# lightkurve/lightkurve

Hardware: NVIDIA H100
Metric: lombscargle_freqbins_x_cadences_per_s (higher is better)
Workload: dtype f32 spreading + FFT, f64 phase (nufft)

## Files before the change

lightkurve_b200/csrc/ls_nufft.cu:

```cuda
#include <algorithm>

#include "common.cuh"
#include "ls_common.cuh"
#include "nufft_core.h"
#include "nufft_v2.cuh"

namespace lkb {

using nufft::Cad;

namespace {

constexpr int GL_NQ = 48;
struct GlNodes {
  double x[GL_NQ], w[GL_NQ];
};

__global__ void nufft_cad_kernel(const double* __restrict__ t, int64_t N, double df, int64_t M, int w,
                                 Cad* __restrict__ cad, int* __restrict__ unsorted) {
  const int64_t n = (int64_t)blockIdx.x * blockDim.x + threadIdx.x;
  if (n >= N) return;
  cad[n] = nufft::cad_entry(t[n], df, M, w);
  if (n > 0 && t[n] < t[n - 1]) *unsorted = 1;
  if (t[n] < 0.0) *unsorted = 1;
// ... 307 lines not shown
    for (int64_t s0 = n_lo; s0 < n_hi; s0 += 256) {
      float v0[8], v1[8];
#pragma unroll
      for (int q = 0; q < 8; ++q) {
        const int64_t n = s0 + lane + 32 * q;
        v0[q] = (n < n_hi) ? y0[n] : 0.0f;
        v1[q] = (n < n_hi) ? y1[n] : 0.0f;
      }
      __syncthreads();
      {
        const int64_t n = s0 + threadIdx.x;
#pragma unroll
        for (int r = 0; r < LOWR; ++r)
          sD[r][threadIdx.x] = (r < nr && n < n_hi) ? D[(int64_t)(r0 + r) * Npad + n] : make_float2(0.f, 0.f);
      }
      __syncthreads();
#pragma unroll
      for (int q = 0; q < 8; ++q) {
#pragma unroll
        for (int r = 0; r < LOWR; ++r) {
          const float2 d = sD[r][lane + 32 * q];
          ac0[r] = fmaf(v0[q], d.x, ac0[r]); as0[r] = fmaf(v0[q], d.y, as0[r]);
          ac1[r] = fmaf(v1[q], d.x, ac1[r]); as1[r] = fmaf(v1[q], d.y, as1[r]);
        }
      }
    }
#pragma unroll
    for (int r = 0; r < LOWR; ++r) {
      if (r < nr) {
        const double c0v = warp_sum((double)ac0[r]), s0v = warp_sum((double)as0[r]);
        const double c1v = warp_sum((double)ac1[r]), s1v = warp_sum((double)as1[r]);
        if (lane == 0) {
          if (b0 < B) { atomicAdd(acc + ((int64_t)b0 * F_low + r0 + r) * 2, c0v); atomicAdd(acc + ((int64_t)b0 * F_low + r0 + r) * 2 + 1, s0v); }
          if (b1 < B) { atomicAdd(acc + ((int64_t)b1 * F_low + r0 + r) * 2, c1v); atomicAdd(acc + ((int64_t)b1 * F_low + r0 + r) * 2 + 1, s1v); }
        }
      }
    }
  }
}
__global__ void nufft2_lowfinish_kernel(const double* __restrict__ acc, int B, int F_low, int64_t F, int64_t N,
                                        const float4* __restrict__ rot, const float2* __restrict__ rot2,
                                        const float* __restrict__ ysum, int normalization, float scale,
                                        float* __restrict__ power, unsigned* __restrict__ peak) {
  const int e = (int)(blockIdx.x * blockDim.x + threadIdx.x);
  if (e >= B * F_low) return;
  const int b = e / F_low, k = e - b * F_low;
  const float pw = ls_epilogue_shared((float)acc[2 * (int64_t)e], (float)acc[2 * (int64_t)e + 1], rot[k], rot2[k], ysum[b],
                                      (float)N, LKB_LS_NORM_PSD_RAW, 1.0f, true);
  power[(int64_t)b * F + k] = v2_normalise(pw, (float)N, normalization, scale);
  if (peak && pw > 0.0f) atomicMax(peak + b, __float_as_uint(pw));
}

constexpr int LOWX_PER = 8;
__global__ void __launch_bounds__(256)
nufft2_lowacc_kernel(const int* __restrict__ list, V2Count nc, const double* __restrict__ t, int64_t N,
                     const float* __restrict__ yc, int64_t ystride, const double* __restrict__ freq, int F_low,
                     double* __restrict__ accW, double* __restrict__ accY, double* __restrict__ accS) {
  const int ntr = v2_count(nc, 0);
  if (ntr <= 0) return;
  const int k = (int)blockIdx.x, lane = threadIdx.x & 31;
  const int64_t n0 = (int64_t)blockIdx.y * (256 * LOWX_PER) + threadIdx.x;
  const double fr = freq[k];
  double sn[LOWX_PER], cs[LOWX_PER];
  double ws = 0.0, wc = 0.0, wcc = 0.0, wsc = 0.0;
#pragma unroll
  for (int q = 0; q < LOWX_PER; ++q) {
    const int64_t n = n0 + (int64_t)q * 256;
    sn[q] = 0.0; cs[q] = 0.0;
    if (n < N) {
      ls_sincos_cycles_f64(fr * t[n], sn[q], cs[q]);
      ws += sn[q]; wc += cs[q]; wcc += cs[q] * cs[q]; wsc += sn[q] * cs[q];
    }
  }
  ws = warp_sum(ws); wc = warp_sum(wc); wcc = warp_sum(wcc); wsc = warp_sum(wsc);
  if (lane == 0) {
    atomicAdd(accW + 4 * k + 0, ws); atomicAdd(accW + 4 * k + 1, wc);
    atomicAdd(accW + 4 * k + 2, wcc); atomicAdd(accW + 4 * k + 3, wsc);
  }
  for (int i = 0; i < ntr; ++i) {
    const float* y = yc + (int64_t)list[nc.base + i] * ystride;
    double sh = 0.0, ch = 0.0, sy = 0.0;
#pragma unroll
    for (int q = 0; q < LOWX_PER; ++q) {
      const int64_t n = n0 + (int64_t)q * 256;
      const double v = (n < N) ? (double)y[n] : 0.0;
      sh = fma(v, sn[q], sh);
      ch = fma(v, cs[q], ch);
      sy += v;
    }
    sh = warp_sum(sh); ch = warp_sum(ch);
    if (k == 0) sy = warp_sum(sy);
    if (lane == 0) {
      atomicAdd(accY + ((int64_t)i * F_low + k) * 2 + 0, sh);
      atomicAdd(accY + ((int64_t)i * F_low + k) * 2 + 1, ch);
      if (k == 0) atomicAdd(accS + i, sy);
    }
  }
}
__global__ void nufft2_lowexact_finish_kernel(const int* __restrict__ list, V2Count nc, const double* __restrict__ accW,
                                              const double* __restrict__ accY, const double* __restrict__ accS,
                                              int F_low, int64_t F, int64_t N, int normalization, float scale,
                                              float* __restrict__ power) {
  const int ntr = v2_count(nc, 0);
  const int e = (int)(blockIdx.x * blockDim.x + threadIdx.x);
  if (e >= ntr * F_low) return;
  const int i = e / F_low, k = e - i * F_low;
  LsSums<double> d;
  d.sh = accY[2 * (int64_t)e]; d.ch = accY[2 * (int64_t)e + 1];
  d.s = accW[4 * k]; d.c = accW[4 * k + 1]; d.cc = accW[4 * k + 2]; d.sc = accW[4 * k + 3];
  power[(int64_t)list[nc.base + i] * F + k] =
      ls_normalize(ls_power_from_sums(d, (double)N, accS[i]), (double)N, normalization, (double)scale);
}

__global__ void __launch_bounds__(128)
nufft2_verify_kernel(const float2* __restrict__ Zn, int p, const float2* __restrict__ dec, int64_t k0, int64_t F,
                     int64_t k_lo, const double* __restrict__ t, int64_t N, const float* __restrict__ yc, int64_t ystride,
                     const double* __restrict__ freq, int nv, float fault, unsigned* __restrict__ worst) {
  const int warp = threadIdx.x >> 5, lane = threadIdx.x & 31;
  const unsigned job = blockIdx.x * (blockDim.x >> 5) + warp;
  unsigned h = job * 2654435761u + 12345u;
  h ^= h >> 15; h *= 2246822519u; h ^= h >> 13;
  const int64_t b = h % (unsigned)nv;
  const int64_t k = k_lo + (int64_t)((h >> 8) % (unsigned)(F - k_lo));
  const float* y = yc + b * ystride;
  const double fr = freq[k];
  double c = 0.0, s = 0.0, l1 = 0.0;
  for (int64_t i = lane; i < N; i += 32) {
    double sn, cs;
    ls_sincos_cycles_f64(fr * t[i], sn, cs);
    const double v = (double)y[i];
    c += v * cs;
    s += v * sn;
    l1 += fabs(v);
  }
  c = warp_sum(c);
  s = warp_sum(s);
  l1 = warp_sum(l1);
  if (lane == 0) {
    const int64_t M = (int64_t)1 << p, Mh = M >> 1, kk = k0 + k;
    const float2 g1 = Zn[b * Mh + kk], g2 = Zn[b * Mh + ((Mh - kk) & (Mh - 1))];
    const float2 E = make_float2(0.5f * (g1.x + g2.x), 0.5f * (g1.y - g2.y));
    const float2 O = make_float2(0.5f * (g1.y + g2.y), 0.5f * (g2.x - g1.x));
    double wsn, wcs;
    sincospi(2.0 * (double)kk / (double)M, &wsn, &wcs);
    const float2 G = make_float2(E.x + (float)wcs * O.x - (float)wsn * O.y, E.y + (float)wcs * O.y + (float)wsn * O.x);
    const float2 got = nufft::cmul(G, dec[k]);
    const double dev = fmax(fabs((double)got.x * (double)fault - c), fabs((double)got.y * (double)fault - s));
    const double units = dev / (1e-7 * fmax(l1, 1e-300));
// ... 273 lines not shown
    LKB_TRY(ws_get_t<float2>(ws_alt ? WS_OUT5 : WS_I, std::max((size_t)B * cells, verify ? (size_t)4 * Mh : (size_t)0), &G));
    unsigned* d_worst = nullptr;
    if (verify) LKB_TRY(ws_get_t<unsigned>(ws_alt ? WS_OUT7 : WS_OUT6, 1, &d_worst));
    const int ptc = V2_LOG_TILE - (p - 1 - V2_PB);
    if (prof) prof_begin(st);
    constexpr int LCS = 8;
    LKB_LAUNCH(dim3(blocks_for((int64_t)cells, 256), (unsigned)((B + LCS - 1) / LCS)), 256, st, nufft2_spread_kernel<LCS>)(
        pl.fge, pl.cad, pl.Wt, d_yc, ystride, B, w, p, ptc, pl.n1max, G);
    LKB_LAUNCH_CHECK();
    LKB_TRY(v2_cols(G, T, p, pl.n1max, B, pl.tb, st));
    const float esc_ratio = escalate_ratio();
    unsigned* d_peak = nullptr;
    int* d_list = nullptr;
    if (esc_ratio > 0.0f && F_low < F) {
      LKB_TRY(ws_get_t<unsigned>(ws_alt ? WS_Y3 : WS_Y2, (size_t)2 * B + 1, &d_peak));
      d_list = reinterpret_cast<int*>(d_peak + B);
      LKB_CUDA_CHECK(cudaMemsetAsync(d_peak, 0, sizeof(unsigned) * ((size_t)B + 1), st));
    }
    V2Finish fa;
    fa.ftab = pl.ftab; fa.k0 = k0; fa.F = F; fa.k_lo = F_low; fa.ysum = d_ysumf; fa.Nf = (float)N;
    fa.normalization = normalization; fa.scale = (float)norm_scale; fa.power = d_pow;
    fa.peak = d_peak; fa.lcmap = nullptr; fa.log2M = p;
    if (F_low < F) LKB_TRY(v2_rows(T, p, B, pl.tb, &fa, (float2*)nullptr, 0, st));
    if (F_low > 0) {
      double* acc = nullptr;
      LKB_TRY(ws_get_t<double>(ws_alt ? WS_X4 : WS_X3, (size_t)B * F_low * 2, &acc));
      LKB_CUDA_CHECK(cudaMemsetAsync(acc, 0, sizeof(double) * (size_t)B * F_low * 2, st));
      const int groups = (B + 15) / 16;
      const int64_t slice = 2048;
      LKB_LAUNCH(dim3((unsigned)groups, (unsigned)((N + slice - 1) / slice)), 256, st, nufft2_lowrows_kernel)(
          pl.lowD, N, pl.Npad, d_yc, ystride, B, (int)F_low, slice, acc);
      LKB_LAUNCH_CHECK();
      LKB_LAUNCH(blocks_for((int64_t)B * F_low, 256), 256, st, nufft2_lowfinish_kernel)(
          acc, B, (int)F_low, F, N, d_rot, d_rot2, d_ysumf, normalization, (float)norm_scale, d_pow, d_peak);
      LKB_LAUNCH_CHECK();
    }
    if (d_peak) {
      LKB_LAUNCH(blocks_for(B, 256), 256, st, nufft2_flag_kernel)(d_peak, d_absmax, B, (float)N, esc_ratio, d_list, d_list + 1,
                                                                pl.esc_total);
      LKB_LAUNCH_CHECK();
      int cap_max = 1024;
      if (const char* e = getenv("LKB_NUFFT_ESCALATE_CAP")) cap_max = std::max(1, atoi(e));
      const int cap = std::min(B, cap_max), gy = std::min(cap, 32);
      const size_t lowlen = F_low > 0 ? (size_t)F_low * 4 + (size_t)cap * F_low * 2 + cap : 0;
      double *Gbuf = nullptr;
      double2* Td = nullptr;
      LKB_TRY(ws_get_t<double>(ws_alt ? WS_Y6 : WS_Y4, 2 * (size_t)cap * cells + lowlen, &Gbuf));
      LKB_TRY(ws_get_t<double2>(ws_alt ? WS_Y7 : WS_Y5, (size_t)cap * Mh, &Td));
      double2* Gd = reinterpret_cast<double2*>(Gbuf);
      double* accW = Gbuf + 2 * (size_t)cap * cells;
      double* accY = accW + (size_t)F_low * 4;
      double* accS = accY + (size_t)cap * F_low * 2;
      const int* lst = d_list + 1;
      for (int base = 0; base < B; base += cap) {
        const V2Count nc = {d_list, base, cap};
        LKB_LAUNCH(dim3(blocks_for((int64_t)cells, 256), (unsigned)gy), 256, st, nufft2_spread_list_kernel)(
            pl.fge, pl.cad, pl.Wtd, d_yc, ystride, lst, w, p, ptc, pl.n1max, Gd, nc);
        LKB_LAUNCH_CHECK();
        LKB_TRY(v2_cols(Gd, Td, p, pl.n1max, gy, pl.tbd, st, nc));
        V2Finish fd = fa;
        fd.peak = nullptr;
        fd.lcmap = lst;
        LKB_TRY(v2_rows(Td, p, gy, pl.tbd, &fd, (double2*)nullptr, 0, st, nc));
        if (F_low > 0) {
          LKB_CUDA_CHECK(cudaMemsetAsync(accW, 0, sizeof(double) * lowlen, st));
          LKB_LAUNCH(dim3((unsigned)F_low, blocks_for(N, 256 * LOWX_PER)), 256, st, nufft2_lowacc_kernel)(
              lst, nc, d_t, N, d_yc, ystride, d_freq, (int)F_low, accW, accY, accS);
          LKB_LAUNCH_CHECK();
          LKB_LAUNCH(blocks_for((int64_t)cap * F_low, 256), 256, st, nufft2_lowexact_finish_kernel)(
              lst, nc, accW, accY, accS, (int)F_low, F, N, normalization, (float)norm_scale, d_pow);
          LKB_LAUNCH_CHECK();
        }
      }
    }
    if (prof) prof_end(st);
    if (verify) {
      const int nv = std::min(B, 4);
      const int nk2 = (int)((k0 + F) >> (p - 1 - V2_PB)) + 1;
      LKB_TRY(v2_rows(T, p, nv, pl.tb, (const V2Finish*)nullptr, G, nk2, st));
      const char* fe = getenv("LKB_NUFFT_INJECT_FAULT");
      LKB_CUDA_CHECK(cudaMemsetAsync(d_worst, 0, sizeof(unsigned), st));
      LKB_LAUNCH(16, 128, st, nufft2_verify_kernel)(G, p, pl.dec, k0, F, F_low, d_t, N, d_yc, ystride, d_freq, nv,
                                                  fe ? (float)atof(fe) : 1.0f, d_worst);
      LKB_LAUNCH_CHECK();
      unsigned h_worst = 0;
      LKB_CUDA_CHECK(cudaMemcpyAsync(&h_worst, d_worst, sizeof(unsigned), cudaMemcpyDeviceToHost, st));
      LKB_CUDA_CHECK(cudaStreamSynchronize(st));
      if (h_worst > 100u) {
        set_error("NUFFT self-check failed: transform deviates from the direct sums by %u x 1e-7 sum|y|", h_worst);
        return LKB_E_VERIFY;
      }
    }
    return LKB_OK;
  }
  float2 *Za = nullptr, *Zb = nullptr;
  LKB_TRY(ws_get_t<float2>(ws_alt ? WS_OUT4 : WS_H, (size_t)npairs * M, &Za));
  LKB_TRY(ws_get_t<float2>(ws_alt ? WS_OUT5 : WS_I, (size_t)npairs * M, &Zb));
  unsigned* d_worst = nullptr;
  if (verify) LKB_TRY(ws_get_t<unsigned>(ws_alt ? WS_OUT7 : WS_OUT6, 1, &d_worst));

  int group = npairs;
  if (const char* e = getenv("LKB_NUFFT_GROUP_MB")) {
    const double mb = atof(e);
    if (mb > 0.0) {
      const double per_pair = 2.0 * (double)M * sizeof(float2) / 1048576.0;
      group = (int)fmax(1.0, floor(mb / per_pair));
      if (group > npairs) group = npairs;
    }
  }
  if (prof) prof_begin(st);
// ... 614 lines not shown
```

lightkurve_b200/csrc/nufft_v2.cuh:

```cuda
#pragma once
#include "nufft_core.h"

namespace lkb {
namespace {

using nufft::V2_PB;
using nufft::V2_THREADS;
using nufft::V2_TILE;
constexpr int V2_LOG_TILE = 13;
static_assert((1 << V2_LOG_TILE) == V2_TILE, "tile size");
constexpr int V2_BC = 1 << V2_PB;
constexpr int V2_R = V2_TILE / (2 * V2_BC);
constexpr int V2_LSB = V2_BC + V2_BC / 16 + 1;
constexpr int V2R_P_MIN = V2_PB + 4 + 1, V2R_P_MAX = V2_PB + 13 + 1;

__host__ __device__ constexpr int v2_radix(int plog, int idx) {
  return (idx < plog / 4) ? 16 : ((idx == plog / 4 && (plog % 4)) ? (1 << (plog % 4)) : 0);
}
__host__ __device__ constexpr int v2_log2i(int r) { return r == 16 ? 4 : r == 8 ? 3 : r == 4 ? 2 : r == 2 ? 1 : 0; }
__device__ __forceinline__ int v2_skew(int a) { return a + (a >> 4); }
template <int nb>
__host__ __device__ constexpr int v2_in_off(int r) {
  return (nb % 16 == 0) ? r * (nb + nb / 16) : r * nb + ((r * nb) >> 4);
}

template <class CT>
__global__ void nufft2_tables_kernel(int pa, int pb, int ph, CT* __restrict__ tw_a, CT* __restrict__ tw_b,
                                     CT* __restrict__ t_hi, CT* __restrict__ t_lo) {
  const int la = nufft::v2_pass_table_len(pa), lb = nufft::v2_pass_table_len(pb), pl = nufft::v2_log2_lo(ph);
  const int nlo = 1 << pl, nhi = 1 << (ph - pl);
  int e = (int)(blockIdx.x * blockDim.x + threadIdx.x);
  int64_t num = 0, den = 1;
  CT* dst = nullptr;
  if (e < la) { nufft::v2_pass_table_entry(pa, e, &num, &den); dst = tw_a + e; }
  else if ((e -= la) < lb) { nufft::v2_pass_table_entry(pb, e, &num, &den); dst = tw_b + e; }
  else if ((e -= lb) < nhi) { num = e; den = nhi; dst = t_hi + e; }
  else if ((e -= nhi) < nlo) { num = e; den = (int64_t)1 << ph; dst = t_lo + e; }
  else return;
  double sn, cs;
  sincospi(2.0 * (double)num / (double)den, &sn, &cs);
  typedef typename nufft::CplxOf<CT>::real RT;
  *dst = nufft::CplxOf<CT>::mk((RT)cs, (RT)sn);
}

template <class RT>
__global__ void nufft2_weights_kernel(const double* __restrict__ t, int64_t N, double df, int64_t M, int w, double beta,
                                      RT* __restrict__ Wt) {
  const int64_t e = (int64_t)blockIdx.x * blockDim.x + threadIdx.x;
  if (e >= N * w) return;
  const int64_t n = e / w;
  const int q = (int)(e - n * w);
  const double x = df * t[n] * (double)M + (double)nufft::grid_shift(w);
  const double i0 = ceil(x - 0.5 * (double)w);
  const double z = (i0 + (double)q - x) * (2.0 / (double)w);
  const double s2 = 1.0 - z * z;
  Wt[e] = (s2 > 0.0) ? (RT)exp(beta * (sqrt(s2) - 1.0)) : (RT)0.0;
}

__device__ __forceinline__ int64_t v2_zcell_of(int64_t e, int ptc, int n1max) {
  const int64_t j = e & (((int64_t)1 << ptc) - 1), rest = e >> ptc;
  const int64_t n1 = rest % n1max, c = rest / n1max;
  return (n1 << V2_PB) + (c << ptc) + j;
}

template <int LCS>
__global__ void __launch_bounds__(256)
nufft2_spread_kernel(const int32_t* __restrict__ first_ge, const nufft::Cad* __restrict__ cad,
                     const float* __restrict__ Wt, const float* __restrict__ y, int64_t ystride, int B, int w, int p,
                     int ptc, int n1max, float2* __restrict__ G) {
  const int64_t cells = (int64_t)n1max << V2_PB;
  const int64_t e = (int64_t)blockIdx.x * blockDim.x + threadIdx.x;
  if (e >= cells) return;
  const int64_t M = (int64_t)1 << p, m = 2 * v2_zcell_of(e, ptc, n1max);
  const int lc0 = (int)blockIdx.y * LCS;
  const float* yr[LCS];
#pragma unroll
  for (int q = 0; q < LCS; ++q) {
    int b = lc0 + q;
    if (b > B - 1) b = B - 1;
    yr[q] = y + (int64_t)b * ystride;
  }
  float a0[LCS], a1[LCS];
#pragma unroll
  for (int q = 0; q < LCS; ++q) { a0[q] = 0.0f; a1[q] = 0.0f; }
  const int64_t L = nufft::table_len(M, w);
  for (int wrap = 0; wrap < 2; ++wrap) {
    const int64_t mm = m + (int64_t)wrap * M;
    if (mm + 1 >= L) break;
    int64_t lo_c = mm - w + 1, hi_c = mm + 2;
    if (lo_c < 0) lo_c = 0;
    if (hi_c > L - 1) hi_c = L - 1;
    const int32_t na = first_ge[lo_c], nb = first_ge[hi_c];
    for (int32_t n = na; n < nb; ++n) {
      const int tap = (int)(mm - (int64_t)cad[n].i0);
      const float* wr = Wt + (int64_t)n * w;
      const float w0 = (tap >= 0) ? wr[tap] : 0.0f;
      const float w1 = (tap + 1 < w) ? wr[tap + 1] : 0.0f;
#pragma unroll
      for (int q = 0; q < LCS; ++q) {
        const float v = yr[q][n];
        a0[q] = fmaf(w0, v, a0[q]);
        a1[q] = fmaf(w1, v, a1[q]);
      }
    }
  }
#pragma unroll
  for (int q = 0; q < LCS; ++q)
    if (lc0 + q < B) G[(int64_t)(lc0 + q) * cells + e] = make_float2(a0[q], a1[q]);
}

template <int PLOG, int LS, int IDX, int NS, class CT = float2>
__device__ __forceinline__ void v2_pass_t(CT* buf, const CT* __restrict__ tw, int nz = 1 << 30) {
  constexpr int R = v2_radix(PLOG, IDX);
  if constexpr (R != 0) {
    constexpr int LR = v2_log2i(R), NB = 16 / R, PNB = PLOG - LR, nb = 1 << PNB;
    constexpr bool WIDE = nb > V2_THREADS;
    static_assert(WIDE || (V2_THREADS % nb) == 0, "geometry");
    const int t = (int)threadIdx.x;
    CT u[NB][R];
    int base_in[NB];
#pragma unroll
    for (int q = 0; q < NB; ++q) {
      int line, i;
      if constexpr (WIDE) { line = 0; i = t + V2_THREADS * q; }
      else { line = (t >> PNB) + ((V2_THREADS * q) >> PNB); i = t & (nb - 1); }
      base_in[q] = line * LS + ((nb % 16 == 0) ? v2_skew(i) : i);
#pragma unroll
      for (int r = 0; r < R; ++r)
        u[q][r] = (IDX > 0 || r * nb < nz) ? buf[base_in[q] + v2_in_off<nb>(r)] : nufft::CplxOf<CT>::mk(0, 0);
    }
    __syncthreads();
#pragma unroll
    for (int q = 0; q < NB; ++q) {
      int line, i;
      if constexpr (WIDE) { line = 0; i = t + V2_THREADS * q; }
      else { line = (t >> PNB) + ((V2_THREADS * q) >> PNB); i = t & (nb - 1); }
      const int k = i & (NS - 1);
      if constexpr (NS > 1) {
#pragma unroll
        for (int r = 1; r < R; ++r) u[q][r] = nufft::cmul(u[q][r], tw[r * NS + k]);
      }
      nufft::SmallDft<R, CT>::run(u[q]);
      const int j = ((i - k) << LR) + k;
      const int base_out = line * LS + ((NS == 1) ? (j + i) : v2_skew(j));
#pragma unroll
      for (int r = 0; r < R; ++r) buf[base_out + ((NS == 1) ? r : r * (NS + NS / 16))] = u[q][r];
    }
    __syncthreads();
    v2_pass_t<PLOG, LS, IDX + 1, NS * R, CT>(buf, tw + ((IDX > 0) ? R * NS : 0));
  }
}

struct V2Count {
  const int* count;
  int base, cap;
};
__device__ __forceinline__ int v2_count(const V2Count nc, int grid_y) {
  if (!nc.count) return grid_y;
  const int n = *nc.count - nc.base;
  return n < 0 ? 0 : (n > nc.cap ? nc.cap : n);
}

template <int PA, class CT>
__device__ __forceinline__ void v2_cols_one(CT* buf, const CT* __restrict__ G, CT* __restrict__ T, int n1max,
                                            const CT* __restrict__ tw_a, const CT* __restrict__ t_hi,
                                            const CT* __restrict__ t_lo, const int64_t lc) {
  constexpr int A = 1 << PA, PTC = V2_LOG_TILE - PA, TC = 1 << PTC, LS = A + A / 16 + 1, C = V2_BC / TC;
  constexpr int JW = TC < 32 ? TC : 32, RW = V2_THREADS / JW, CG = TC / JW;
  constexpr int LJW = JW == 32 ? 5 : JW == 16 ? 4 : JW == 8 ? 3 : JW == 4 ? 2 : JW == 2 ? 1 : 0;
  static_assert((1 << LJW) == JW && RW % 16 == 0, "geometry");
  const int t = (int)threadIdx.x, c = (int)blockIdx.x;
  const int jl = t & (JW - 1), nl = t >> LJW;
  const int nvalid = n1max << PTC;
  const CT* Gp = G + (lc * C + c) * (int64_t)nvalid;
  const int s_base = jl * LS + v2_skew(nl), g_base = nl * TC + jl;
  constexpr int NB1 = A / v2_radix(PA, 0);
  const int nz = ((n1max + NB1 - 1) / NB1) * NB1;
#pragma unroll
  for (int u = 0; u < 16; ++u) {
    const int cg = u % CG, nbk = u / CG;
    if (nbk * RW < nz) {
      const int idx = g_base + nbk * RW * TC + cg * JW;
      buf[s_base + cg * JW * LS + nbk * (RW + RW / 16)] = (idx < nvalid) ? Gp[idx] : nufft::CplxOf<CT>::mk(0, 0);
    }
  }
  __syncthreads();
  v2_pass_t<PA, LS, 0, 1, CT>(buf, tw_a, nz);
  CT* Tp = T + (lc * C + c) * (int64_t)V2_TILE;
  const int ph = PA + V2_PB, pl = nufft::v2_log2_lo(ph);
  const unsigned Mmask = (1u << ph) - 1u, lmask = (1u << pl) - 1u;
#pragma unroll
  for (int u = 0; u < 16; ++u) {
    const int cg = u % CG, nbk = u / CG;
    const int k1 = nl + nbk * RW, n2 = c * TC + jl + cg * JW;
    const unsigned q = ((unsigned)n2 * (unsigned)k1) & Mmask;
    const CT wq = nufft::cmul(t_hi[q >> pl], t_lo[q & lmask]);
    Tp[g_base + nbk * RW * TC + cg * JW] = nufft::cmul(buf[s_base + cg * JW * LS + nbk * (RW + RW / 16)], wq);
  }
}
template <int PA, class CT = float2>
__global__ void __launch_bounds__(V2_THREADS, sizeof(CT) == 8 ? 2 : 1)
nufft2_cols_kernel(const CT* __restrict__ G, CT* __restrict__ T, int n1max, const CT* __restrict__ tw_a,
                   const CT* __restrict__ t_hi, const CT* __restrict__ t_lo) {
  LKB_DYN_SMEM(CT, buf);
  v2_cols_one<PA, CT>(buf, G, T, n1max, tw_a, t_hi, t_lo, (int64_t)blockIdx.y);
}
template <int PA>
__global__ void __launch_bounds__(V2_THREADS, 1)
nufft2_cols_list_kernel(const double2* __restrict__ G, double2* __restrict__ T, int n1max,
                        const double2* __restrict__ tw_a, const double2* __restrict__ t_hi,
                        const double2* __restrict__ t_lo, V2Count nc) {
  LKB_DYN_SMEM(double2, buf);
  const int64_t ntr = v2_count(nc, (int)gridDim.y);
  for (int64_t lc = blockIdx.y; lc < ntr; lc += gridDim.y) {
    __syncthreads();
    v2_cols_one<PA, double2>(buf, G, T, n1max, tw_a, t_hi, t_lo, lc);
  }
}

struct V2FTab {
  float4 d;
  float4 c;
};
struct V2Finish {
  const V2FTab* ftab;
  int64_t k0, F, k_lo;
  const float* ysum;
  float Nf;
  int normalization;
  float scale;
  float* power;
  unsigned* peak;
  const int* lcmap;
  int log2M;
};

__device__ __forceinline__ float v2_normalise(float pw, float Nf, int normalization, float scale) {
  if (normalization == LKB_LS_NORM_PSD_SCALE) return pw * scale;
  if (normalization == LKB_LS_NORM_AMPLITUDE) return sqrtf(pw * (4.0f / Nf));
  return pw;
}
__device__ __forceinline__ float v2_finish_pw(float2 g1, float2 g2, const V2FTab tb, float ysum, int64_t, int) {
  const float ex = 0.5f * (g1.x + g2.x), ey = 0.5f * (g1.y - g2.y);
  const float ox = 0.5f * (g1.y + g2.y), oy = 0.5f * (g2.x - g1.x);
  const float yc = ex * tb.d.x - ey * tb.d.y + ox * tb.d.z - oy * tb.d.w - ysum * tb.c.x;
  const float ys = ex * tb.d.y + ey * tb.d.x + ox * tb.d.w + oy * tb.d.z - ysum * tb.c.y;
  return yc * yc * tb.c.z + ys * ys * tb.c.w;
}
__device__ __forceinline__ float v2_finish_pw(double2 g1, double2 g2, const V2FTab tb, float ysum, int64_t kk, int log2M) {
  const double ex = 0.5 * (g1.x + g2.x), ey = 0.5 * (g1.y - g2.y);
  const double ox = 0.5 * (g1.y + g2.y), oy = 0.5 * (g2.x - g1.x);
  double sw, cw;
  sincospi(ldexp((double)kk, 1 - log2M), &sw, &cw);
  const double gx = ex + cw * ox - sw * oy, gy = ey + cw * oy + sw * ox;
  const double yc = gx * (double)tb.d.x - gy * (double)tb.d.y - (double)ysum * (double)tb.c.x;
  const double ys = gx * (double)tb.d.y + gy * (double)tb.d.x - (double)ysum * (double)tb.c.y;
  return (float)(yc * yc * (double)tb.c.z + ys * ys * (double)tb.c.w);
}

template <int PA, int MODE, class CT>
__device__ __forceinline__ void v2_rows_one(CT* buf, const CT* __restrict__ T, const CT* __restrict__ tw_b,
                                            const V2Finish& fa, CT* __restrict__ Zout, int nk2_keep, const int64_t lc,
                                            const int lc_base, const int g) {
  constexpr int A = 1 << PA, PTC = V2_LOG_TILE - PA, TC = 1 << PTC, R = V2_R, LS = V2_LSB, Bc = V2_BC;
  const int t = (int)threadIdx.x;
  const bool last = g == (A / (2 * R)) - 1;
  const int64_t Mh = (int64_t)1 << (PA + V2_PB);
  auto slot_k1 = [&](int s) -> int {
    const int h = s >> 3, r = s & (R - 1);
    if (h == 0) return 1 + g * R + r;
    if (last && r == 0) return 0;
    return A - (g + 1) * R + r;
  };
  const CT* Tp = T + lc * Mh;
#pragma unroll
  for (int u = 0; u < 16; ++u) {
    const int e = t + V2_THREADS * u;
    const int j = e & (TC - 1), r = (e >> PTC) & (R - 1), h = (e >> (PTC + 3)) & 1, c = e >> (PTC + 4);
    const int s = h * R + r;
    buf[s * LS + v2_skew((c << PTC) + j)] = Tp[(((c << PA) + slot_k1(s)) << PTC) + j];
  }
  __syncthreads();
  v2_pass_t<V2_PB, LS, 0, 1, CT>(buf, tw_b);
  const int s = t & (2 * R - 1), h = s >> 3, r = s & (R - 1), k1 = slot_k1(s);
  if (MODE == 2) {
    const int keep = nk2_keep < Bc / 2 ? nk2_keep : Bc / 2;
    for (int q = t >> 4; q < 2 * keep; q += V2_THREADS / 16) {
      const int k2 = q < keep ? q : Bc - 2 * keep + q;
      Zout[lc * Mh + k1 + ((int64_t)k2 << PA)] = buf[s * LS + v2_skew(k2)];
    }
  } else {
  int ps = (1 - h) * R + (R - 1 - r);
  bool row0 = false;
  if (last && h == 0 && r == R - 1) ps = s;
  if (last && h == 1 && r == 0) { ps = s; row0 = true; }
  int64_t nK2 = ((fa.k0 + fa.F - 1) >> PA) + 1;
  if (nK2 > Bc) nK2 = Bc;
  const int64_t lcd = fa.lcmap ? (int64_t)fa.lcmap[lc_base + lc] : lc;
  const float ys0 = fa.ysum[lcd];
  float* prow = fa.power + lcd * fa.F;
  const int64_t jbase = (int64_t)k1 - fa.k0;
  float pmax = 0.0f;
  constexpr int KSTEP = V2_THREADS / 16, UB = 4;
  for (int k2b = t >> 4; k2b < (int)nK2; k2b += KSTEP * UB) {
    V2FTab tb[UB];
    int64_t jj[UB];
    bool valid[UB];
#pragma unroll
    for (int u = 0; u < UB; ++u) {
      const int k2 = k2b + KSTEP * u;
      jj[u] = jbase + ((int64_t)k2 << PA);
      valid[u] = k2 < (int)nK2 && jj[u] >= fa.k_lo && jj[u] < fa.F;
      if (valid[u]) tb[u] = fa.ftab[jj[u]];
    }
#pragma unroll
    for (int u = 0; u < UB; ++u) {
      if (!valid[u]) continue;
      const int k2 = k2b + KSTEP * u;
      const int pi = row0 ? ((Bc - k2) & (Bc - 1)) : (Bc - 1 - k2);
      const CT g1 = buf[s * LS + v2_skew(k2)], g2 = buf[ps * LS + v2_skew(pi)];
      const float pw = v2_finish_pw(g1, g2, tb[u], ys0, fa.k0 + jj[u], fa.log2M);
      pmax = fmaxf(pmax, pw);
      prow[jj[u]] = v2_normalise(pw, fa.Nf, fa.normalization, fa.scale);
    }
  }
  if (fa.peak) {
#pragma unroll
    for (int o = 16; o > 0; o >>= 1) pmax = fmaxf(pmax, __shfl_xor_sync(0xffffffffu, pmax, o));
    if ((t & 31) == 0 && pmax > 0.0f) atomicMax(fa.peak + lcd, __float_as_uint(pmax));
  }
  }
}

template <int PA, int MODE, class CT = float2>
__global__ void __launch_bounds__(V2_THREADS, sizeof(CT) == 8 ? 2 : 1)
nufft2_rows_kernel(const CT* __restrict__ T, const CT* __restrict__ tw_b, V2Finish fa, CT* __restrict__ Zout,
                   int nk2_keep) {
  LKB_DYN_SMEM(CT, buf);
  v2_rows_one<PA, MODE, CT>(buf, T, tw_b, fa, Zout, nk2_keep, (int64_t)blockIdx.y, 0, (int)blockIdx.x);
}
template <int PA>
__global__ void __launch_bounds__(V2_THREADS, 1)
nufft2_rows_list_kernel(const double2* __restrict__ T, const double2* __restrict__ tw_b, V2Finish fa, V2Count nc) {
  LKB_DYN_SMEM(double2, buf);
  const int64_t ntr = v2_count(nc, (int)gridDim.y);
  for (int64_t lc = blockIdx.y; lc < ntr; lc += gridDim.y) {
    __syncthreads();
    v2_rows_one<PA, 1, double2>(buf, T, tw_b, fa, nullptr, 0, lc, nc.base, (int)blockIdx.x);
  }
}

__global__ void nufft2_flag_kernel(const unsigned* __restrict__ peak, const float* __restrict__ absmax, int B, float Nf,
                                   float ratio, int* __restrict__ count, int* __restrict__ list, int* __restrict__ total) {
  const int b = (int)(blockIdx.x * blockDim.x + threadIdx.x);
  bool f = false;
  if (b < B) {
    const float amp = sqrtf(__uint_as_float(peak[b]) * (4.0f / Nf));
    f = absmax[b] > ratio * amp;
  }
  const unsigned bal = __ballot_sync(0xffffffffu, f);
  if (bal) {
    int base = 0;
    if ((threadIdx.x & 31) == 0) {
      base = atomicAdd(count, __popc(bal));
      if (total) atomicAdd(total, __popc(bal));
    }
    base = __shfl_sync(0xffffffffu, base, 0);
    if (f) list[base + __popc(bal & ((1u << (threadIdx.x & 31)) - 1u))] = b;
  }
}

__global__ void __launch_bounds__(256)
nufft2_spread_list_kernel(const int32_t* __restrict__ first_ge, const nufft::Cad* __restrict__ cad,
                          const double* __restrict__ Wt, const float* __restrict__ y, int64_t ystride,
                          const int* __restrict__ list, int w, int p, int ptc, int n1max, double2* __restrict__ G,
                          V2Count nc) {
  const int64_t cells = (int64_t)n1max << V2_PB;
  const int64_t e = (int64_t)blockIdx.x * blockDim.x + threadIdx.x;
  if (e >= cells) return;
  const int64_t M = (int64_t)1 << p, m = 2 * v2_zcell_of(e, ptc, n1max);
  const int ntr = v2_count(nc, (int)gridDim.y);
  for (int i = (int)blockIdx.y; i < ntr; i += (int)gridDim.y) {
  const float* yr = y + (int64_t)list[nc.base + i] * ystride;
  double a0 = 0.0, a1 = 0.0;
  const int64_t L = nufft::table_len(M, w);
  for (int wrap = 0; wrap < 2; ++wrap) {
    const int64_t mm = m + (int64_t)wrap * M;
    if (mm + 1 >= L) break;
    int64_t lo_c = mm - w + 1, hi_c = mm + 2;
    if (lo_c < 0) lo_c = 0;
    if (hi_c > L - 1) hi_c = L - 1;
    const int32_t na = first_ge[lo_c], nb = first_ge[hi_c];
    for (int32_t n = na; n < nb; ++n) {
      const int tap = (int)(mm - (int64_t)cad[n].i0);
      const double* wr = Wt + (int64_t)n * w;
      const double w0 = (tap >= 0) ? wr[tap] : 0.0, w1 = (tap + 1 < w) ? wr[tap + 1] : 0.0;
      const double v = (double)yr[n];
      a0 = fma(w0, v, a0);
      a1 = fma(w1, v, a1);
    }
  }
  G[(int64_t)i * cells + e] = make_double2(a0, a1);
  }
}

inline unsigned v2_blocks_for(int64_t n, int per) { return (unsigned)((n + per - 1) / per); }

template <class CT>
struct V2TablesT {
  const CT *tw_a, *tw_b, *t_hi, *t_lo;
};
typedef V2TablesT<float2> V2Tables;
typedef V2TablesT<double2> V2TablesD;
template <class CT>
inline int v2_tables(int p, int slot, cudaStream_t st, V2TablesT<CT>* out) {
  const int ph = p - 1, pa = ph - V2_PB, pl = nufft::v2_log2_lo(ph);
  const int la = nufft::v2_pass_table_len(pa), lb = nufft::v2_pass_table_len(V2_PB), nhi = 1 << (ph - pl), nlo = 1 << pl;
  CT* base = nullptr;
  LKB_TRY(ws_get_t<CT>(slot, (size_t)(la + lb + nhi + nlo + 4), &base));
  CT *tw_a = base, *tw_b = base + la, *t_hi = tw_b + lb, *t_lo = t_hi + nhi;
  LKB_LAUNCH(v2_blocks_for(la + lb + nhi + nlo, 256), 256, st, nufft2_tables_kernel<CT>)(pa, V2_PB, ph, tw_a, tw_b, t_hi, t_lo);
  LKB_LAUNCH_CHECK();
  out->tw_a = tw_a; out->tw_b = tw_b; out->t_hi = t_hi; out->t_lo = t_lo;
  return LKB_OK;
}
inline int v2_n1max(int p, int64_t i0_last, int w) {
  const int64_t M = (int64_t)1 << p, A = (M / 2) >> V2_PB;
  const int64_t reach = i0_last + w + 1;
  if (reach >= M) return (int)A;
  const int64_t n = ((reach + 1) / 2 + V2_BC - 1) >> V2_PB;
  return (int)(n < 1 ? 1 : (n > A ? A : n));
}
inline bool v2_supported(int p) { return p >= V2R_P_MIN && p <= V2R_P_MAX; }

template <int PA, class CT>
int v2_cols_pa(const CT* G, CT* T, int n1max, int B, const V2TablesT<CT>& tb, cudaStream_t st, V2Count nc) {
  constexpr int A = 1 << PA, TC = V2_TILE / A;
  const size_t smem = (size_t)TC * (A + A / 16 + 1) * sizeof(CT);
  const dim3 grid((unsigned)(V2_BC / TC), (unsigned)B);
  if constexpr (sizeof(CT) == 16) {
    if (nc.count) {
      LKB_CUDA_CHECK(cudaFuncSetAttribute(nufft2_cols_list_kernel<PA>, cudaFuncAttributeMaxDynamicSharedMemorySize, (int)smem));
      LKB_LAUNCH_SMEM(grid, V2_THREADS, smem, st, nufft2_cols_list_kernel<PA>)(G, T, n1max, tb.tw_a, tb.t_hi, tb.t_lo, nc);
      LKB_LAUNCH_CHECK();
      return LKB_OK;
    }
  }
  LKB_CUDA_CHECK(cudaFuncSetAttribute(nufft2_cols_kernel<PA, CT>, cudaFuncAttributeMaxDynamicSharedMemorySize, (int)smem));
  LKB_LAUNCH_SMEM(grid, V2_THREADS, smem, st, nufft2_cols_kernel<PA, CT>)(G, T, n1max, tb.tw_a, tb.t_hi, tb.t_lo);
  LKB_LAUNCH_CHECK();
  return LKB_OK;
}
template <int PA, class CT>
int v2_rows_pa(const CT* T, int B, const V2TablesT<CT>& tb, const V2Finish* fa, CT* Zout, int nk2_keep, cudaStream_t st,
               V2Count nc) {
  const size_t smem = (size_t)(2 * V2_R) * V2_LSB * sizeof(CT);
  const dim3 grid((unsigned)((1 << PA) / (2 * V2_R)), (unsigned)B);
  if constexpr (sizeof(CT) == 16) {
    if (nc.count && fa) {
      LKB_CUDA_CHECK(cudaFuncSetAttribute(nufft2_rows_list_kernel<PA>, cudaFuncAttributeMaxDynamicSharedMemorySize, (int)smem));
      LKB_LAUNCH_SMEM(grid, V2_THREADS, smem, st, nufft2_rows_list_kernel<PA>)(T, tb.tw_b, *fa, nc);
      LKB_LAUNCH_CHECK();
      return LKB_OK;
    }
  }
  LKB_CUDA_CHECK(cudaFuncSetAttribute(nufft2_rows_kernel<PA, 1, CT>, cudaFuncAttributeMaxDynamicSharedMemorySize, (int)smem));
  LKB_CUDA_CHECK(cudaFuncSetAttribute(nufft2_rows_kernel<PA, 2, CT>, cudaFuncAttributeMaxDynamicSharedMemorySize, (int)smem));
  if (fa) LKB_LAUNCH_SMEM(grid, V2_THREADS, smem, st, nufft2_rows_kernel<PA, 1, CT>)(T, tb.tw_b, *fa, nullptr, 0);
  else LKB_LAUNCH_SMEM(grid, V2_THREADS, smem, st, nufft2_rows_kernel<PA, 2, CT>)(T, tb.tw_b, V2Finish(), Zout, nk2_keep);
  LKB_LAUNCH_CHECK();
  return LKB_OK;
}
#define V2_DISPATCH_PA(pa, CALL)                                                                       \
  switch (pa) {                                                                                         \
    case 4: return CALL(4); case 5: return CALL(5); case 6: return CALL(6); case 7: return CALL(7);      \
    case 8: return CALL(8); case 9: return CALL(9); case 10: return CALL(10); case 11: return CALL(11);  \
    case 12: return CALL(12); case 13: return CALL(13);                                                  \
    default: set_error("NUFFT v2: fine grid of 2^%d cells out of range", (pa) + V2_PB + 1); return LKB_E_UNSUPPORTED; \
  }
template <class CT>
inline int v2_cols(const CT* G, CT* T, int p, int n1max, int B, const V2TablesT<CT>& tb, cudaStream_t st,
                   V2Count nc = V2Count{nullptr, 0, 0}) {
#define V2_CALL(PA) v2_cols_pa<PA, CT>(G, T, n1max, B, tb, st, nc)
  V2_DISPATCH_PA(p - 1 - V2_PB, V2_CALL)
#undef V2_CALL
}
template <class CT>
inline int v2_rows(const CT* T, int p, int B, const V2TablesT<CT>& tb, const V2Finish* fa, CT* Zout, int nk2_keep,
                   cudaStream_t st, V2Count nc = V2Count{nullptr, 0, 0}) {
#define V2_CALL(PA) v2_rows_pa<PA, CT>(T, B, tb, fa, Zout, nk2_keep, st, nc)
  V2_DISPATCH_PA(p - 1 - V2_PB, V2_CALL)
#undef V2_CALL
}

}
}
```

Baseline: 1611000 billion.

## Batch light curves in escalation spread/lowacc and shrink f64 FFT tiles

```diff
diff --git a/lightkurve_b200/csrc/ls_nufft.cu b/lightkurve_b200/csrc/ls_nufft.cu
--- a/lightkurve_b200/csrc/ls_nufft.cu
+++ b/lightkurve_b200/csrc/ls_nufft.cu
@@ -383,6 +383,7 @@
 }
 
 constexpr int LOWX_PER = 8;
+constexpr int LOWX_LC = 4;
 __global__ void __launch_bounds__(256)
 nufft2_lowacc_kernel(const int* __restrict__ list, V2Count nc, const double* __restrict__ t, int64_t N,
                      const float* __restrict__ yc, int64_t ystride, const double* __restrict__ freq, int F_low,
@@ -408,23 +409,36 @@
     atomicAdd(accW + 4 * k + 0, ws); atomicAdd(accW + 4 * k + 1, wc);
     atomicAdd(accW + 4 * k + 2, wcc); atomicAdd(accW + 4 * k + 3, wsc);
   }
-  for (int i = 0; i < ntr; ++i) {
-    const float* y = yc + (int64_t)list[nc.base + i] * ystride;
-    double sh = 0.0, ch = 0.0, sy = 0.0;
+  for (int i0 = 0; i0 < ntr; i0 += LOWX_LC) {
+    float v[LOWX_LC][LOWX_PER];
 #pragma unroll
-    for (int q = 0; q < LOWX_PER; ++q) {
-      const int64_t n = n0 + (int64_t)q * 256;
-      const double v = (n < N) ? (double)y[n] : 0.0;
-      sh = fma(v, sn[q], sh);
-      ch = fma(v, cs[q], ch);
-      sy += v;
-    }
-    sh = warp_sum(sh); ch = warp_sum(ch);
-    if (k == 0) sy = warp_sum(sy);
-    if (lane == 0) {
-      atomicAdd(accY + ((int64_t)i * F_low + k) * 2 + 0, sh);
-      atomicAdd(accY + ((int64_t)i * F_low + k) * 2 + 1, ch);
-      if (k == 0) atomicAdd(accS + i, sy);
+    for (int j = 0; j < LOWX_LC; ++j) {
+      const float* y = yc + (int64_t)list[nc.base + ((i0 + j < ntr) ? i0 + j : ntr - 1)] * ystride;
+#pragma unroll
+      for (int q = 0; q < LOWX_PER; ++q) {
+        const int64_t n = n0 + (int64_t)q * 256;
+        v[j][q] = (n < N) ? y[n] : 0.0f;
+      }
+    }
+#pragma unroll
+    for (int j = 0; j < LOWX_LC; ++j) {
+      const int i = i0 + j;
+      if (i >= ntr) break;
+      double sh = 0.0, ch = 0.0, sy = 0.0;
+#pragma unroll
+      for (int q = 0; q < LOWX_PER; ++q) {
+        const double vq = (double)v[j][q];
+        sh = fma(vq, sn[q], sh);
+        ch = fma(vq, cs[q], ch);
+        sy += vq;
+      }
+      sh = warp_sum(sh); ch = warp_sum(ch);
+      if (k == 0) sy = warp_sum(sy);
+      if (lane == 0) {
+        atomicAdd(accY + ((int64_t)i * F_low + k) * 2 + 0, sh);
+        atomicAdd(accY + ((int64_t)i * F_low + k) * 2 + 1, ch);
+        if (k == 0) atomicAdd(accS + i, sy);
+      }
     }
   }
 }
@@ -804,10 +818,11 @@
       double* accY = accW + (size_t)F_low * 4;
       double* accS = accY + (size_t)cap * F_low * 2;
       const int* lst = d_list + 1;
+      const int ptc_d = v2_log_tile(p - 1 - V2_PB, true) - (p - 1 - V2_PB);
       for (int base = 0; base < B; base += cap) {
         const V2Count nc = {d_list, base, cap};
-        LKB_LAUNCH(dim3(blocks_for((int64_t)cells, 256), (unsigned)gy), 256, st, nufft2_spread_list_kernel)(
-            pl.fge, pl.cad, pl.Wtd, d_yc, ystride, lst, w, p, ptc, pl.n1max, Gd, nc);
+        LKB_LAUNCH(dim3(blocks_for((int64_t)cells, 256), (unsigned)((gy + LCS_D - 1) / LCS_D)), 256, st,
+                   nufft2_spread_list_kernel)(pl.fge, pl.cad, pl.Wtd, d_yc, ystride, lst, w, p, ptc_d, pl.n1max, Gd, nc);
         LKB_LAUNCH_CHECK();
         LKB_TRY(v2_cols(Gd, Td, p, pl.n1max, gy, pl.tbd, st, nc));
         V2Finish fd = fa;
diff --git a/lightkurve_b200/csrc/nufft_v2.cuh b/lightkurve_b200/csrc/nufft_v2.cuh
--- a/lightkurve_b200/csrc/nufft_v2.cuh
+++ b/lightkurve_b200/csrc/nufft_v2.cuh
@@ -18,6 +18,7 @@
   return (idx < plog / 4) ? 16 : ((idx == plog / 4 && (plog % 4)) ? (1 << (plog % 4)) : 0);
 }
 __host__ __device__ constexpr int v2_log2i(int r) { return r == 16 ? 4 : r == 8 ? 3 : r == 4 ? 2 : r == 2 ? 1 : 0; }
+__host__ __device__ constexpr int v2_log_tile(int pa, bool dbl) { return (dbl && pa <= 12) ? 12 : V2_LOG_TILE; }
 __device__ __forceinline__ int v2_skew(int a) { return a + (a >> 4); }
 template <int nb>
 __host__ __device__ constexpr int v2_in_off(int r) {
@@ -109,21 +110,21 @@
     if (lc0 + q < B) G[(int64_t)(lc0 + q) * cells + e] = make_float2(a0[q], a1[q]);
 }
 
-template <int PLOG, int LS, int IDX, int NS, class CT = float2>
+template <int PLOG, int LS, int IDX, int NS, class CT = float2, int NT = V2_THREADS>
 __device__ __forceinline__ void v2_pass_t(CT* buf, const CT* __restrict__ tw, int nz = 1 << 30) {
   constexpr int R = v2_radix(PLOG, IDX);
   if constexpr (R != 0) {
     constexpr int LR = v2_log2i(R), NB = 16 / R, PNB = PLOG - LR, nb = 1 << PNB;
-    constexpr bool WIDE = nb > V2_THREADS;
-    static_assert(WIDE || (V2_THREADS % nb) == 0, "geometry");
+    constexpr bool WIDE = nb > NT;
+    static_assert(WIDE || (NT % nb) == 0, "geometry");
     const int t = (int)threadIdx.x;
     CT u[NB][R];
     int base_in[NB];
 #pragma unroll
     for (int q = 0; q < NB; ++q) {
       int line, i;
-      if constexpr (WIDE) { line = 0; i = t + V2_THREADS * q; }
-      else { line = (t >> PNB) + ((V2_THREADS * q) >> PNB); i = t & (nb - 1); }
+      if constexpr (WIDE) { line = 0; i = t + NT * q; }
+      else { line = (t >> PNB) + ((NT * q) >> PNB); i = t & (nb - 1); }
       base_in[q] = line * LS + ((nb % 16 == 0) ? v2_skew(i) : i);
 #pragma unroll
       for (int r = 0; r < R; ++r)
@@ -133,8 +134,8 @@
 #pragma unroll
     for (int q = 0; q < NB; ++q) {
       int line, i;
-      if constexpr (WIDE) { line = 0; i = t + V2_THREADS * q; }
-      else { line = (t >> PNB) + ((V2_THREADS * q) >> PNB); i = t & (nb - 1); }
+      if constexpr (WIDE) { line = 0; i = t + NT * q; }
+      else { line = (t >> PNB) + ((NT * q) >> PNB); i = t & (nb - 1); }
       const int k = i & (NS - 1);
       if constexpr (NS > 1) {
 #pragma unroll
@@ -147,7 +148,7 @@
       for (int r = 0; r < R; ++r) buf[base_out + ((NS == 1) ? r : r * (NS + NS / 16))] = u[q][r];
     }
     __syncthreads();
-    v2_pass_t<PLOG, LS, IDX + 1, NS * R, CT>(buf, tw + ((IDX > 0) ? R * NS : 0));
+    v2_pass_t<PLOG, LS, IDX + 1, NS * R, CT, NT>(buf, tw + ((IDX > 0) ? R * NS : 0));
   }
 }
 
@@ -161,12 +162,13 @@
   return n < 0 ? 0 : (n > nc.cap ? nc.cap : n);
 }
 
-template <int PA, class CT>
+template <int PA, class CT, int LOGT = V2_LOG_TILE>
 __device__ __forceinline__ void v2_cols_one(CT* buf, const CT* __restrict__ G, CT* __restrict__ T, int n1max,
                                             const CT* __restrict__ tw_a, const CT* __restrict__ t_hi,
                                             const CT* __restrict__ t_lo, const int64_t lc) {
-  constexpr int A = 1 << PA, PTC = V2_LOG_TILE - PA, TC = 1 << PTC, LS = A + A / 16 + 1, C = V2_BC / TC;
-  constexpr int JW = TC < 32 ? TC : 32, RW = V2_THREADS / JW, CG = TC / JW;
+  constexpr int NT = (1 << LOGT) / 16;
+  constexpr int A = 1 << PA, PTC = LOGT - PA, TC = 1 << PTC, LS = A + A / 16 + 1, C = V2_BC / TC;
+  constexpr int JW = TC < NT / 16 ? TC : NT / 16, RW = NT / JW, CG = TC / JW;
   constexpr int LJW = JW == 32 ? 5 : JW == 16 ? 4 : JW == 8 ? 3 : JW == 4 ? 2 : JW == 2 ? 1 : 0;
   static_assert((1 << LJW) == JW && RW % 16 == 0, "geometry");
   const int t = (int)threadIdx.x, c = (int)blockIdx.x;
@@ -185,8 +187,8 @@
     }
   }
   __syncthreads();
-  v2_pass_t<PA, LS, 0, 1, CT>(buf, tw_a, nz);
-  CT* Tp = T + (lc * C + c) * (int64_t)V2_TILE;
+  v2_pass_t<PA, LS, 0, 1, CT, NT>(buf, tw_a, nz);
+  CT* Tp = T + (lc * C + c) * (int64_t)(1 << LOGT);
   const int ph = PA + V2_PB, pl = nufft::v2_log2_lo(ph);
   const unsigned Mmask = (1u << ph) - 1u, lmask = (1u << pl) - 1u;
 #pragma unroll
@@ -205,8 +207,15 @@
   LKB_DYN_SMEM(CT, buf);
   v2_cols_one<PA, CT>(buf, G, T, n1max, tw_a, t_hi, t_lo, (int64_t)blockIdx.y);
 }
-template <int PA>
-__global__ void __launch_bounds__(V2_THREADS, 1)
+template <int PA, int LOGT>
+__device__ __noinline__ void v2_cols_list_one(double2* buf, const double2* __restrict__ G, double2* __restrict__ T,
+                                              int n1max, const double2* __restrict__ tw_a,
+                                              const double2* __restrict__ t_hi, const double2* __restrict__ t_lo,
+                                              const int64_t lc) {
+  v2_cols_one<PA, double2, LOGT>(buf, G, T, n1max, tw_a, t_hi, t_lo, lc);
+}
+template <int PA, int LOGT = v2_log_tile(PA, true)>
+__global__ void __launch_bounds__((1 << LOGT) / 16, LOGT < V2_LOG_TILE ? 2 : 1)
 nufft2_cols_list_kernel(const double2* __restrict__ G, double2* __restrict__ T, int n1max,
                         const double2* __restrict__ tw_a, const double2* __restrict__ t_hi,
                         const double2* __restrict__ t_lo, V2Count nc) {
@@ -214,7 +223,7 @@
   const int64_t ntr = v2_count(nc, (int)gridDim.y);
   for (int64_t lc = blockIdx.y; lc < ntr; lc += gridDim.y) {
     __syncthreads();
-    v2_cols_one<PA, double2>(buf, G, T, n1max, tw_a, t_hi, t_lo, lc);
+    v2_cols_list_one<PA, LOGT>(buf, G, T, n1max, tw_a, t_hi, t_lo, lc);
   }
 }
 
@@ -258,16 +267,18 @@
   return (float)(yc * yc * (double)tb.c.z + ys * ys * (double)tb.c.w);
 }
 
-template <int PA, int MODE, class CT>
+template <int PA, int MODE, class CT, int LOGT = V2_LOG_TILE>
 __device__ __forceinline__ void v2_rows_one(CT* buf, const CT* __restrict__ T, const CT* __restrict__ tw_b,
                                             const V2Finish& fa, CT* __restrict__ Zout, int nk2_keep, const int64_t lc,
                                             const int lc_base, const int g) {
-  constexpr int A = 1 << PA, PTC = V2_LOG_TILE - PA, TC = 1 << PTC, R = V2_R, LS = V2_LSB, Bc = V2_BC;
+  constexpr int NT = (1 << LOGT) / 16, R = (1 << LOGT) / (2 * V2_BC), LR = v2_log2i(R);
+  constexpr int A = 1 << PA, PTC = LOGT - PA, TC = 1 << PTC, LS = V2_LSB, Bc = V2_BC;
+  static_assert((1 << LR) == R, "geometry");
   const int t = (int)threadIdx.x;
   const bool last = g == (A / (2 * R)) - 1;
   const int64_t Mh = (int64_t)1 << (PA + V2_PB);
   auto slot_k1 = [&](int s) -> int {
-    const int h = s >> 3, r = s & (R - 1);
+    const int h = s >> LR, r = s & (R - 1);
     if (h == 0) return 1 + g * R + r;
     if (last && r == 0) return 0;
     return A - (g + 1) * R + r;
@@ -275,17 +286,18 @@
   const CT* Tp = T + lc * Mh;
 #pragma unroll
   for (int u = 0; u < 16; ++u) {
-    const int e = t + V2_THREADS * u;
-    const int j = e & (TC - 1), r = (e >> PTC) & (R - 1), h = (e >> (PTC + 3)) & 1, c = e >> (PTC + 4);
+    const int e = t + NT * u;
+    const int j = e & (TC - 1), r = (e >> PTC) & (R - 1), h = (e >> (PTC + LR)) & 1, c = e >> (PTC + LR + 1);
     const int s = h * R + r;
     buf[s * LS + v2_skew((c << PTC) + j)] = Tp[(((c << PA) + slot_k1(s)) << PTC) + j];
   }
   __syncthreads();
-  v2_pass_t<V2_PB, LS, 0, 1, CT>(buf, tw_b);
-  const int s = t & (2 * R - 1), h = s >> 3, r = s & (R - 1), k1 = slot_k1(s);
+  v2_pass_t<V2_PB, LS, 0, 1, CT, NT>(buf, tw_b);
+  constexpr int KSTEP = NT / (2 * R);
+  const int s = t & (2 * R - 1), h = s >> LR, r = s & (R - 1), k1 = slot_k1(s);
   if (MODE == 2) {
     const int keep = nk2_keep < Bc / 2 ? nk2_keep : Bc / 2;
-    for (int q = t >> 4; q < 2 * keep; q += V2_THREADS / 16) {
+    for (int q = t >> (LR + 1); q < 2 * keep; q += KSTEP) {
       const int k2 = q < keep ? q : Bc - 2 * keep + q;
       Zout[lc * Mh + k1 + ((int64_t)k2 << PA)] = buf[s * LS + v2_skew(k2)];
     }
@@ -301,8 +313,8 @@
   float* prow = fa.power + lcd * fa.F;
   const int64_t jbase = (int64_t)k1 - fa.k0;
   float pmax = 0.0f;
-  constexpr int KSTEP = V2_THREADS / 16, UB = 4;
-  for (int k2b = t >> 4; k2b < (int)nK2; k2b += KSTEP * UB) {
+  constexpr int UB = 4;
+  for (int k2b = t >> (LR + 1); k2b < (int)nK2; k2b += KSTEP * UB) {
     V2FTab tb[UB];
     int64_t jj[UB];
     bool valid[UB];
@@ -339,14 +351,20 @@
   LKB_DYN_SMEM(CT, buf);
   v2_rows_one<PA, MODE, CT>(buf, T, tw_b, fa, Zout, nk2_keep, (int64_t)blockIdx.y, 0, (int)blockIdx.x);
 }
-template <int PA>
-__global__ void __launch_bounds__(V2_THREADS, 1)
+template <int PA, int LOGT>
+__device__ __noinline__ void v2_rows_list_one(double2* buf, const double2* __restrict__ T,
+                                              const double2* __restrict__ tw_b, const V2Finish fa, const int64_t lc,
+                                              const int lc_base) {
+  v2_rows_one<PA, 1, double2, LOGT>(buf, T, tw_b, fa, nullptr, 0, lc, lc_base, (int)blockIdx.x);
+}
+template <int PA, int LOGT = v2_log_tile(PA, true)>
+__global__ void __launch_bounds__((1 << LOGT) / 16, LOGT < V2_LOG_TILE ? 2 : 1)
 nufft2_rows_list_kernel(const double2* __restrict__ T, const double2* __restrict__ tw_b, V2Finish fa, V2Count nc) {
   LKB_DYN_SMEM(double2, buf);
   const int64_t ntr = v2_count(nc, (int)gridDim.y);
   for (int64_t lc = blockIdx.y; lc < ntr; lc += gridDim.y) {
     __syncthreads();
-    v2_rows_one<PA, 1, double2>(buf, T, tw_b, fa, nullptr, 0, lc, nc.base, (int)blockIdx.x);
+    v2_rows_list_one<PA, LOGT>(buf, T, tw_b, fa, lc, nc.base);
   }
 }
 
@@ -370,6 +388,7 @@
   }
 }
 
+constexpr int LCS_D = 4;
 __global__ void __launch_bounds__(256)
 nufft2_spread_list_kernel(const int32_t* __restrict__ first_ge, const nufft::Cad* __restrict__ cad,
                           const double* __restrict__ Wt, const float* __restrict__ y, int64_t ystride,
@@ -379,28 +398,40 @@
   const int64_t e = (int64_t)blockIdx.x * blockDim.x + threadIdx.x;
   if (e >= cells) return;
   const int64_t M = (int64_t)1 << p, m = 2 * v2_zcell_of(e, ptc, n1max);
-  const int ntr = v2_count(nc, (int)gridDim.y);
-  for (int i = (int)blockIdx.y; i < ntr; i += (int)gridDim.y) {
-  const float* yr = y + (int64_t)list[nc.base + i] * ystride;
-  double a0 = 0.0, a1 = 0.0;
   const int64_t L = nufft::table_len(M, w);
-  for (int wrap = 0; wrap < 2; ++wrap) {
-    const int64_t mm = m + (int64_t)wrap * M;
-    if (mm + 1 >= L) break;
-    int64_t lo_c = mm - w + 1, hi_c = mm + 2;
-    if (lo_c < 0) lo_c = 0;
-    if (hi_c > L - 1) hi_c = L - 1;
-    const int32_t na = first_ge[lo_c], nb = first_ge[hi_c];
-    for (int32_t n = na; n < nb; ++n) {
-      const int tap = (int)(mm - (int64_t)cad[n].i0);
-      const double* wr = Wt + (int64_t)n * w;
-      const double w0 = (tap >= 0) ? wr[tap] : 0.0, w1 = (tap + 1 < w) ? wr[tap + 1] : 0.0;
-      const double v = (double)yr[n];
-      a0 = fma(w0, v, a0);
-      a1 = fma(w1, v, a1);
-    }
-  }
-  G[(int64_t)i * cells + e] = make_double2(a0, a1);
+  const int ntr = v2_count(nc, (int)gridDim.y * LCS_D);
+  for (int i0 = (int)blockIdx.y * LCS_D; i0 < ntr; i0 += (int)gridDim.y * LCS_D) {
+    const float* yr[LCS_D];
+#pragma unroll
+    for (int q = 0; q < LCS_D; ++q) {
+      const int i = (i0 + q < ntr) ? i0 + q : ntr - 1;
+      yr[q] = y + (int64_t)list[nc.base + i] * ystride;
+    }
+    double a0[LCS_D], a1[LCS_D];
+#pragma unroll
+    for (int q = 0; q < LCS_D; ++q) { a0[q] = 0.0; a1[q] = 0.0; }
+    for (int wrap = 0; wrap < 2; ++wrap) {
+      const int64_t mm = m + (int64_t)wrap * M;
+      if (mm + 1 >= L) break;
+      int64_t lo_c = mm - w + 1, hi_c = mm + 2;
+      if (lo_c < 0) lo_c = 0;
+      if (hi_c > L - 1) hi_c = L - 1;
+      const int32_t na = first_ge[lo_c], nb = first_ge[hi_c];
+      for (int32_t n = na; n < nb; ++n) {
+        const int tap = (int)(mm - (int64_t)cad[n].i0);
+        const double* wr = Wt + (int64_t)n * w;
+        const double w0 = (tap >= 0) ? wr[tap] : 0.0, w1 = (tap + 1 < w) ? wr[tap + 1] : 0.0;
+#pragma unroll
+        for (int q = 0; q < LCS_D; ++q) {
+          const double v = (double)yr[q][n];
+          a0[q] = fma(w0, v, a0[q]);
+          a1[q] = fma(w1, v, a1[q]);
+        }
+      }
+    }
+#pragma unroll
+    for (int q = 0; q < LCS_D; ++q)
+      if (i0 + q < ntr) G[(int64_t)(i0 + q) * cells + e] = make_double2(a0[q], a1[q]);
   }
 }
 
@@ -435,39 +466,34 @@
 
 template <int PA, class CT>
 int v2_cols_pa(const CT* G, CT* T, int n1max, int B, const V2TablesT<CT>& tb, cudaStream_t st, V2Count nc) {
-  constexpr int A = 1 << PA, TC = V2_TILE / A;
+  constexpr int LOGT = v2_log_tile(PA, sizeof(CT) == 16), A = 1 << PA, TC = (1 << LOGT) / A;
   const size_t smem = (size_t)TC * (A + A / 16 + 1) * sizeof(CT);
   const dim3 grid((unsigned)(V2_BC / TC), (unsigned)B);
   if constexpr (sizeof(CT) == 16) {
-    if (nc.count) {
-      LKB_CUDA_CHECK(cudaFuncSetAttribute(nufft2_cols_list_kernel<PA>, cudaFuncAttributeMaxDynamicSharedMemorySize, (int)smem));
-      LKB_LAUNCH_SMEM(grid, V2_THREADS, smem, st, nufft2_cols_list_kernel<PA>)(G, T, n1max, tb.tw_a, tb.t_hi, tb.t_lo, nc);
-      LKB_LAUNCH_CHECK();
-      return LKB_OK;
-    }
-  }
-  LKB_CUDA_CHECK(cudaFuncSetAttribute(nufft2_cols_kernel<PA, CT>, cudaFuncAttributeMaxDynamicSharedMemorySize, (int)smem));
-  LKB_LAUNCH_SMEM(grid, V2_THREADS, smem, st, nufft2_cols_kernel<PA, CT>)(G, T, n1max, tb.tw_a, tb.t_hi, tb.t_lo);
+    LKB_CUDA_CHECK(cudaFuncSetAttribute(nufft2_cols_list_kernel<PA>, cudaFuncAttributeMaxDynamicSharedMemorySize, (int)smem));
+    LKB_LAUNCH_SMEM(grid, (1 << LOGT) / 16, smem, st, nufft2_cols_list_kernel<PA>)(G, T, n1max, tb.tw_a, tb.t_hi, tb.t_lo, nc);
+  } else {
+    LKB_CUDA_CHECK(cudaFuncSetAttribute(nufft2_cols_kernel<PA, CT>, cudaFuncAttributeMaxDynamicSharedMemorySize, (int)smem));
+    LKB_LAUNCH_SMEM(grid, V2_THREADS, smem, st, nufft2_cols_kernel<PA, CT>)(G, T, n1max, tb.tw_a, tb.t_hi, tb.t_lo);
+  }
   LKB_LAUNCH_CHECK();
   return LKB_OK;
 }
 template <int PA, class CT>
 int v2_rows_pa(const CT* T, int B, const V2TablesT<CT>& tb, const V2Finish* fa, CT* Zout, int nk2_keep, cudaStream_t st,
                V2Count nc) {
-  const size_t smem = (size_t)(2 * V2_R) * V2_LSB * sizeof(CT);
-  const dim3 grid((unsigned)((1 << PA) / (2 * V2_R)), (unsigned)B);
+  constexpr int LOGT = v2_log_tile(PA, sizeof(CT) == 16), R = (1 << LOGT) / (2 * V2_BC);
+  const size_t smem = (size_t)(2 * R) * V2_LSB * sizeof(CT);
+  const dim3 grid((unsigned)((1 << PA) / (2 * R)), (unsigned)B);
   if constexpr (sizeof(CT) == 16) {
-    if (nc.count && fa) {
-      LKB_CUDA_CHECK(cudaFuncSetAttribute(nufft2_rows_list_kernel<PA>, cudaFuncAttributeMaxDynamicSharedMemorySize, (int)smem));
-      LKB_LAUNCH_SMEM(grid, V2_THREADS, smem, st, nufft2_rows_list_kernel<PA>)(T, tb.tw_b, *fa, nc);
-      LKB_LAUNCH_CHECK();
-      return LKB_OK;
-    }
-  }
-  LKB_CUDA_CHECK(cudaFuncSetAttribute(nufft2_rows_kernel<PA, 1, CT>, cudaFuncAttributeMaxDynamicSharedMemorySize, (int)smem));
-  LKB_CUDA_CHECK(cudaFuncSetAttribute(nufft2_rows_kernel<PA, 2, CT>, cudaFuncAttributeMaxDynamicSharedMemorySize, (int)smem));
-  if (fa) LKB_LAUNCH_SMEM(grid, V2_THREADS, smem, st, nufft2_rows_kernel<PA, 1, CT>)(T, tb.tw_b, *fa, nullptr, 0);
-  else LKB_LAUNCH_SMEM(grid, V2_THREADS, smem, st, nufft2_rows_kernel<PA, 2, CT>)(T, tb.tw_b, V2Finish(), Zout, nk2_keep);
+    LKB_CUDA_CHECK(cudaFuncSetAttribute(nufft2_rows_list_kernel<PA>, cudaFuncAttributeMaxDynamicSharedMemorySize, (int)smem));
+    LKB_LAUNCH_SMEM(grid, (1 << LOGT) / 16, smem, st, nufft2_rows_list_kernel<PA>)(T, tb.tw_b, *fa, nc);
+  } else {
+    LKB_CUDA_CHECK(cudaFuncSetAttribute(nufft2_rows_kernel<PA, 1, CT>, cudaFuncAttributeMaxDynamicSharedMemorySize, (int)smem));
+    LKB_CUDA_CHECK(cudaFuncSetAttribute(nufft2_rows_kernel<PA, 2, CT>, cudaFuncAttributeMaxDynamicSharedMemorySize, (int)smem));
+    if (fa) LKB_LAUNCH_SMEM(grid, V2_THREADS, smem, st, nufft2_rows_kernel<PA, 1, CT>)(T, tb.tw_b, *fa, nullptr, 0);
+    else LKB_LAUNCH_SMEM(grid, V2_THREADS, smem, st, nufft2_rows_kernel<PA, 2, CT>)(T, tb.tw_b, V2Finish(), Zout, nk2_keep);
+  }
   LKB_LAUNCH_CHECK();
   return LKB_OK;
 }
```

After: 1665000 billion, median of 6. 3.4% higher.
